# MAGIC-AI4Med/KEEP

Measured on AMD Instinct MI355X. Metric: 224x224 tiles encoded/sec (whole node), higher is better.
Workload: dtype fp16+mxfp4

## Files before the change

keep_amd/csrc/common.h:

```cpp
#pragma once
#include <hip/hip_runtime.h>
#include <stdint.h>

typedef _Float16 f16;
typedef _Float16 f16x2 __attribute__((ext_vector_type(2)));
typedef _Float16 f16x4 __attribute__((ext_vector_type(4)));
typedef _Float16 f16x8 __attribute__((ext_vector_type(8)));
typedef float f32x4 __attribute__((ext_vector_type(4)));
typedef float f32x16 __attribute__((ext_vector_type(16)));

#define KEEP_WAVE 64

__device__ __forceinline__ void split_f16(float x, f16& hi, f16& lo) {
    asm("" : "+v"(x));
    hi = (f16)x;
    lo = (f16)(x - (float)hi);
}

__device__ __forceinline__ unsigned char clip8_fixed(int v) {
    v >>= 22;
    return (unsigned char)(v < 0 ? 0 : (v > 255 ? 255 : v));
}
__device__ __forceinline__ float gelu_erf(float x) {
    return 0.5f * x * (1.0f + erff(x * 0.70710678118654752440f));
}

// ... 365 lines not shown
```

keep_amd/csrc/gemm_f16_v2.hip:

```cpp
#include "gemm_epilogue.h"
#include "quant4.h"

#ifndef KEEP_A_AUX
#define KEEP_A_AUX 0
#endif
#ifndef KEEP_W_AUX
#define KEEP_W_AUX 0
#endif
namespace keepk {

constexpr int V2_BM = 256, V2_BK = 32;

__device__ int g_swz_mask_dummy;
__device__ __forceinline__ int v2_swz(int row, int mask = 3) { return (row >> 2) & mask; }
__device__ __forceinline__ int v2_lds_off(int row, int chunk, int mask = 3) {
    return row * V2_BK + ((chunk ^ v2_swz(row, mask)) << 3);
}

template <int N> __device__ __forceinline__ void wait_vmcnt() { asm volatile("s_waitcnt vmcnt(%0)" ::"n"(N) : "memory"); }

typedef const __attribute__((address_space(1))) void* gptr_t;
typedef __attribute__((address_space(3))) void* lptr_t;

constexpr int v2_waves_per_simd(int BN, int WM, int WN) { return (V2_BM / WM / 32) * (BN / WN / 32) * 16 > 128 ? 1 : 2; }

typedef int v8i __attribute__((ext_vector_type(8)));
typedef unsigned u32x4 __attribute__((ext_vector_type(4)));
constexpr int V2_ST2 = 32768;
constexpr int V2_SC2 = 2048;
constexpr int V2_NST2 = 4;
constexpr int V2_SC2_BASE = V2_NST2 * V2_ST2;
constexpr int V2_G2 = 5;
constexpr int V2_PERS_LDS = 160 * 1024;
constexpr int V2_PERS_LDS_F16 = 96 * 1024 + 8 * 4608;

template <int BN, int WM, int WN, int NSTAGE, int EPI, int COMP = 0, bool PERS = false>
__global__ __launch_bounds__(WM * WN * 64, v2_waves_per_simd(BN, WM, WN))
void gemm_f16_v2_kernel(GemmParams p) {
    static_assert(!PERS || (BN == 256 && NSTAGE == 4 && COMP == 0 && (EPI == EPI_F16 || EPI == EPI_GELU_F16 || EPI == EPI_RESID_LS)),
                  "the persistent walk is written for the plain 256x256 / 4-stage kernel");
    constexpr int V2_THREADS = WM * WN * 64;
    constexpr int BM = V2_BM, BK = V2_BK;
    constexpr int TM = BM / WM / 32;
    constexpr int TN = BN / WN / 32;
    constexpr int SLOTS = BK / 8;
    constexpr int A_ROUNDS = BM * SLOTS / V2_THREADS;
    constexpr int B_ROUNDS = BN * SLOTS / V2_THREADS;
    constexpr int G = A_ROUNDS + B_ROUNDS;
    constexpr int BUF_ELEMS = (BM + BN) * BK;
    extern __shared__ __attribute__((aligned(16))) unsigned char smem_raw[];
    f16* lds = reinterpret_cast<f16*>(smem_raw);

    const int tid = threadIdx.x;
    const int lane = tid & 63;
    const int wave = __builtin_amdgcn_readfirstlane(tid >> 6);
    const int wm = wave / WN, wn = wave % WN;

    const int ntn = p.N / BN;
    const int mtn = (p.M + BM - 1) / BM;
// ... 16 lines not shown
            const int remw = ntn % BW, rr = t - full_tiles;
            tm_ = rr / remw; tn_ = (ntn / BW) * BW + (rr - tm_ * remw);
        }
    };
    int tm, tn;
    tile_of(bidx, tm, tn);
    int m0 = tm * BM;
    int n0 = tn * BN;

    const int swz_mask = (p.ablate & 4) ? 0 : 3;
    const int KT = p.K / BK;
    int a_off[A_ROUNDS], w_off[B_ROUNDS];
#pragma unroll
    for (int r = 0; r < A_ROUNDS; ++r) {
        const int L = r * V2_THREADS + tid;
        const int row = L / SLOTS, c = (L % SLOTS) ^ v2_swz(row, swz_mask);
        a_off[r] = row * BK + c * 8;
    }
#pragma unroll
    for (int r = 0; r < B_ROUNDS; ++r) {
        const int L = r * V2_THREADS + tid;
        const int row = L / SLOTS, c = (L % SLOTS) ^ v2_swz(row, swz_mask);
        w_off[r] = ((n0 & 255) + row) * BK + c * 8;
    }
    int64_t a_tile = (int64_t)(m0 >> 8) * KT * 8192;
    int64_t w_tile = (int64_t)(n0 >> 8) * KT * 8192;
    int tile_cur = bidx, m0_n = 0, n0_n = 0;
    int64_t a_tile_n = 0, w_tile_n = 0;
    bool has_next = false, first_tile = true;

    int kt0 = 0, ktiles = KT;
    if (EPI == EPI_PARTIAL) {
        const int per = (KT + p.ksplit - 1) / p.ksplit;
        kt0 = zsplit * per;
        ktiles = (kt0 + per < KT ? kt0 + per : KT) - kt0;
    }
    const int steps = ktiles * p.nseg;
// ... 41 lines not shown
        f16* sw = sa + BM * BK;
#pragma unroll
        for (int r = 0; r < A_ROUNDS; ++r) {
            unsigned o = (unsigned)a_off[r] * 2u;
            asm volatile("" : "+v"(o));
            __builtin_amdgcn_global_load_lds((gptr_t)(reinterpret_cast<const char*>(ab) + o), (lptr_t)(sa + (r * V2_THREADS + wave * 64) * 8), 16, 0, KEEP_A_AUX);
        }
#pragma unroll
        for (int r = 0; r < B_ROUNDS; ++r) {
            unsigned o = (unsigned)w_off[r] * 2u;
            asm volatile("" : "+v"(o));
            __builtin_amdgcn_global_load_lds((gptr_t)(reinterpret_cast<const char*>(wb) + o), (lptr_t)(sw + (r * V2_THREADS + wave * 64) * 8), 16, 0, KEEP_W_AUX);
        }
    };

    f32x16 acc[TN][TM];
    long long t_start = 0, t_first = 0, t_loop = 0;
#ifdef KEEP_DIAGNOSTICS
    if (p.ablate >> 8) {
        const long long wait = (long long)((blockIdx.x >> 3) & 3) * (p.ablate >> 8) * 1024, t0 = __builtin_readcyclecounter();
        while (__builtin_readcyclecounter() - t0 < wait) __builtin_amdgcn_s_sleep(8);
    }
#endif
    if (p.dbg) t_start = __builtin_readcyclecounter();
  for (;;) {
    if constexpr (PERS) {
        const int tnx = tile_cur + (int)gridDim.x;
        has_next = tnx < nwg;
        int tm2, tn2;
        tile_of(has_next ? tnx : tile_cur, tm2, tn2);
        m0_n = tm2 * BM; n0_n = tn2 * BN;
        a_tile_n = (int64_t)(m0_n >> 8) * KT * 8192;
        w_tile_n = (int64_t)(n0_n >> 8) * KT * 8192;
    }
    const int frow = lane & 31, fhi = lane >> 5;
    f16x8 fw0[TN] = {}, fa0[TM], fw1[TN] = {}, fa1[TM];
    auto read_frags = [&](int st, int ks, f16x8 (&fw)[TN], f16x8 (&fa)[TM]) {
        const f16* sa = lds + st * BUF_ELEMS;
        const f16* sw = sa + BM * BK;
#ifdef KEEP_DIAGNOSTICS
        if (!(p.ablate & 8))
#endif
#pragma unroll
        for (int i = 0; i < TN; ++i)
            fw[i] = *reinterpret_cast<const f16x8*>(sw + v2_lds_off(wn * (TN * 32) + i * 32 + frow, ks * 2 + fhi, swz_mask));
#pragma unroll
        for (int j = 0; j < TM; ++j)
            fa[j] = *reinterpret_cast<const f16x8*>(sa + v2_lds_off(wm * (TM * 32) + j * 32 + frow, ks * 2 + fhi, swz_mask));
    };
    constexpr int HM = (TN * TM == 8) ? 5 : TM;
    auto mfma_head = [&](const f16x8 (&fw)[TN], const f16x8 (&fa)[TM]) {
#pragma unroll
        for (int m = 0; m < HM; ++m)
            acc[m / TM][m % TM] = __builtin_amdgcn_mfma_f32_32x32x16_f16(fw[m / TM], fa[m % TM], acc[m / TM][m % TM], 0, 0, 0);
    };
    auto mfma_tail = [&](const f16x8 (&fw)[TN], const f16x8 (&fa)[TM]) {
#pragma unroll
        for (int m = HM; m < TN * TM; ++m)
            acc[m / TM][m % TM] = __builtin_amdgcn_mfma_f32_32x32x16_f16(fw[m / TM], fa[m % TM], acc[m / TM][m % TM], 0, 0, 0);
    };
    auto mfma_group = [&](const f16x8 (&fw)[TN], const f16x8 (&fa)[TM]) { mfma_head(fw, fa); mfma_tail(fw, fa); };
    const unsigned char* aq = nullptr; const unsigned char* wq = nullptr; const unsigned char* sq = nullptr;
    if constexpr (COMP != 0) {
        aq = p.a_q + (int64_t)(m0 >> 8) * KT * 8192;
        wq = p.w_q + (int64_t)(n0 >> 8) * KT * 8192;
        if constexpr (COMP == 1) sq = (wave < 4 ? p.a_sc + (int64_t)(m0 >> 8) * KT * 512 : p.w_sc + (int64_t)(n0 >> 8) * KT * 512 + 256) + (wave & 3) * 512;
        else sq = (wave < 4 ? p.a_sc + (int64_t)(m0 >> 8) * KT * 512 : p.w_sc + (int64_t)(n0 >> 8) * KT * 512) + (wave & 3) * 256;
    }
    const unsigned char* aq_run = aq; const unsigned char* wq_run = wq; const unsigned char* sq_run = sq;
    auto stage2 = [&](int, int buf) {
        unsigned char* sb = smem_raw + buf * V2_ST2;
        unsigned v4 = lane * 4;
        asm volatile("" : "+v"(v4));
#pragma unroll
        for (int r = 0; r < 2; ++r) {
            unsigned va = COMP == 1 ? (tid >> 8) * 8192 + (tid & 255) * 16 : tid * 16, vw = COMP == 1 ? va + 4096 : va;
// ... 12 lines not shown

    if (PERS && p.dbg && !first_tile) t_start = __builtin_readcyclecounter();
    if (!PERS || first_tile) {
#pragma unroll
        for (int t = 0; t < NSTAGE - 1; ++t)
            if (t < steps) stage(t, t);
        if (steps >= NSTAGE - 1) wait_vmcnt<G * (NSTAGE - 2)>(); else wait_vmcnt<0>();
        __builtin_amdgcn_s_barrier();
        if (p.dbg) t_first = __builtin_readcyclecounter();
        if (NSTAGE - 1 < steps) stage(NSTAGE - 1, NSTAGE - 1);
    } else {
        stage(3, 3);
        if (p.dbg) t_first = t_start;
    }
#pragma unroll
    for (int i = 0; i < TN; ++i)
#pragma unroll
        for (int j = 0; j < TM; ++j)
#pragma unroll
            for (int r = 0; r < 16; ++r) acc[i][j][r] = 0.f;
    read_frags(0, 0, fw0, fa0);

#define KEEP_STEADY_STEP(ISSUE)                                                                                                    \
    {                                                                                                                              \
                                                     \
        mfma_head(fw0, fa0);                                                                                                       \
        KEEP_PIN();                                                                                                                \
        read_frags(s % NSTAGE, 1, fw1, fa1);                                                                                       \
        KEEP_PIN();                                                                                                                \
        mfma_tail(fw0, fa0);                                                                                                       \
        KEEP_PIN();                                                                                                                \
        wait_vmcnt<G * (NSTAGE - 2)>();                                                                                            \
        asm volatile("s_waitcnt lgkmcnt(0)" ::: "memory");                                                                         \
        __builtin_amdgcn_s_barrier();                                                                                              \
        KEEP_PIN();                                                                                                                \
                                                      \
        mfma_head(fw1, fa1);                                                                                                       \
        KEEP_PIN();                                                                                                                \
        ISSUE;                                                                                                                     \
        read_frags((s + 1) % NSTAGE, 0, fw0, fa0);                                                                                 \
        KEEP_PIN();                                                                                                                \
        mfma_tail(fw1, fa1);                                                                                                       \
    }
    int s = 0;
    if constexpr (PRE || PERS) {
        for (; s < steps - NSTAGE; ++s) KEEP_STEADY_STEP(stage(s + NSTAGE, s % NSTAGE))
        if constexpr (PRE) KEEP_STEADY_STEP(stage2(0, 0))
        else KEEP_STEADY_STEP(stage_next(0, 0))
        ++s;
    } else {
        for (; s < steps - (NSTAGE - 1); ++s) KEEP_STEADY_STEP(if (s + NSTAGE < steps) stage(s + NSTAGE, s % NSTAGE))
    }
#undef KEEP_STEADY_STEP
#define KEEP_DRAIN_STEP(WAIT, AFTER)                                                                                               \
    {                                                                                                                              \
        mfma_head(fw0, fa0);                                                                                                       \
        KEEP_PIN();                                                                                                                \
        read_frags(s % NSTAGE, 1, fw1, fa1);                                                                                       \
        KEEP_PIN();                                                                                                                \
        mfma_tail(fw0, fa0);                                                                                                       \
        KEEP_PIN();                                                                                                                \
        wait_vmcnt<WAIT>();                                                                                                        \
        asm volatile("s_waitcnt lgkmcnt(0)" ::: "memory");                                                                         \
        __builtin_amdgcn_s_barrier();                                                                                              \
        KEEP_PIN();                                                                                                                \
        mfma_head(fw1, fa1);                                                                                                       \
        KEEP_PIN();                                                                                                                \
        AFTER;                                                                                                                     \
        read_frags((s + 1) % NSTAGE, 0, fw0, fa0);                                                                                 \
        KEEP_PIN();                                                                                                                \
        mfma_tail(fw1, fa1);                                                                                                       \
    }
    if constexpr (PRE) {
        KEEP_DRAIN_STEP(G + V2_G2, stage2(1, 1))
        ++s;
        KEEP_DRAIN_STEP(2 * V2_G2, stage2(2, 2))
        ++s;
    } else if constexpr (PERS) {
        KEEP_DRAIN_STEP(2 * G, stage_next(1, 1))
        ++s;
        KEEP_DRAIN_STEP(2 * G, stage_next(2, 2))
        ++s;
    } else {
        for (; s < steps - 1; ++s) KEEP_DRAIN_STEP(0, (void)0)
    }
#undef KEEP_DRAIN_STEP
    mfma_head(fw0, fa0);
    KEEP_PIN();
    read_frags(s % NSTAGE, 1, fw1, fa1);
    KEEP_PIN();
    mfma_tail(fw0, fa0);
    mfma_group(fw1, fa1);
#undef KEEP_PIN

    if constexpr (COMP != 0) {
        static_assert(BN == 256 && WM == 2 && WN == 4, "phase 2 is written for the 2 x 4 wave grid of the 256 x 256 tile");
        constexpr int G2 = V2_G2;
        if (p.dbg) t_first = __builtin_readcyclecounter();
        constexpr int FH = COMP == 1 ? 4096 : 8192;
        constexpr int SEC = COMP == 1 ? 8192 : 4096;
        constexpr int SFH = COMP == 1 ? 256 : 512, SSEC = COMP == 1 ? 512 : 256;
        const int NC = COMP == 1 ? p.K >> 7 : p.K >> 6;
        if constexpr (PRE) {
            wait_vmcnt<G2 * (V2_NST2 - 2)>();
            asm volatile("s_waitcnt lgkmcnt(0)" ::: "memory");
            __builtin_amdgcn_s_barrier();
        } else {
            asm volatile("s_waitcnt lgkmcnt(0)" ::: "memory");
            __builtin_amdgcn_s_barrier();
#pragma unroll
            for (int t = 0; t < V2_NST2 - 1; ++t)
                if (t < NC) stage2(t, t);
            if (NC >= V2_NST2 - 1) wait_vmcnt<G2 * (V2_NST2 - 2)>(); else wait_vmcnt<0>();
            __builtin_amdgcn_s_barrier();
        }
        const int a_row = (wm * 128 + frow) * 16, w_row = (wn * 64 + frow) * 16;
        const int asc_off = fhi * SFH + (wm * 32 + frow) * 4, wsc_off = 1024 + fhi * SFH + ((wn >> 1) * 32 + frow) * 4;
        const int wsh = (wn & 1) * 16;
#define KEEP_V8(V_) v8i{(int)(V_).x, (int)(V_).y, (int)(V_).z, (int)(V_).w, 0, 0, 0, 0}
#define KEEP_MX(I, J) \
            if constexpr (COMP == 1) { \
                acc[I][J] = __builtin_amdgcn_mfma_scale_f32_32x32x64_f8f6f4(KEEP_V8(wh[I]), KEEP_V8(ah[J]), acc[I][J], 4, 4, I, swh, J, sah); \
                acc[I][J] = __builtin_amdgcn_mfma_scale_f32_32x32x64_f8f6f4(KEEP_V8(wl[I]), KEEP_V8(al[J]), acc[I][J], 4, 4, I, swl, J, sal); \
            } else { \
                acc[I][J] = __builtin_amdgcn_mfma_scale_f32_32x32x64_f8f6f4(KEEP_V8(wl[I]), KEEP_V8(ah[J]), acc[I][J], 4, 4, I, swl, J, sah); \
                acc[I][J] = __builtin_amdgcn_mfma_scale_f32_32x32x64_f8f6f4(KEEP_V8(wh[I]), KEEP_V8(al[J]), acc[I][J], 4, 4, I, swh, J, sal); \
            }
#define KEEP_CHUNK(ISSUE, WAIT)                                                                                                    \
        {                                                                                                                          \
            const unsigned char* sb = smem_raw + (c & (V2_NST2 - 1)) * V2_ST2;                                                     \
            const unsigned char* ss = smem_raw + V2_SC2_BASE + (c & (V2_NST2 - 1)) * V2_SC2;                                       \
            const unsigned char* sa = sb + fhi * FH;         \
            const unsigned char* sw = sb + 16384 + fhi * FH;                                                                       \
                      \
              \
            u32x4 ah[4], al[4], wh[2], wl[2];                                                                                      \
            _Pragma("unroll") for (int jj = 0; jj < 4; ++jj) {                                                                     \
                ah[jj] = *reinterpret_cast<const u32x4*>(sa + a_row + jj * 512);                                                   \
                al[jj] = *reinterpret_cast<const u32x4*>(sa + SEC + a_row + jj * 512);                                             \
            }                                                                                                                      \
            _Pragma("unroll") for (int ii = 0; ii < 2; ++ii) {                                                                     \
                wh[ii] = *reinterpret_cast<const u32x4*>(sw + w_row + ii * 512);                                                   \
                wl[ii] = *reinterpret_cast<const u32x4*>(sw + SEC + w_row + ii * 512);                                             \
            }                                                                                                                      \
            const int sah = *reinterpret_cast<const int*>(ss + asc_off), sal = *reinterpret_cast<const int*>(ss + asc_off + SSEC); \
            const int swh = (int)(*reinterpret_cast<const unsigned*>(ss + wsc_off) >> wsh),                                        \
                      swl = (int)(*reinterpret_cast<const unsigned*>(ss + wsc_off + SSEC) >> wsh);                                 \
            ISSUE;                                                                     \
            KEEP_MX(0, 0) KEEP_MX(0, 1) KEEP_MX(0, 2) KEEP_MX(0, 3)                                                                \
            KEEP_MX(1, 0) KEEP_MX(1, 1) KEEP_MX(1, 2) KEEP_MX(1, 3)                                                                \
            wait_vmcnt<WAIT>();                                                                          \
            asm volatile("s_waitcnt lgkmcnt(0)" ::: "memory");                                                                     \
            __builtin_amdgcn_s_barrier();                                                                                          \
            __builtin_amdgcn_sched_barrier(0);               \
        }
        int c = 0;
        for (; c < NC - (V2_NST2 - 1); ++c) KEEP_CHUNK(stage2(c + V2_NST2 - 1, (c + V2_NST2 - 1) & (V2_NST2 - 1)), G2 * (V2_NST2 - 2))
#pragma clang loop unroll(disable)
        for (; c < NC; ++c) KEEP_CHUNK((void)0, 0)
#undef KEEP_CHUNK
#undef KEEP_MX
#undef KEEP_V8
    }

    if (p.dbg) t_loop = __builtin_readcyclecounter();

    if constexpr (EPI == EPI_TOP2) {
        const int C = p.top2_c;
        const int slot = (m0 >> 8) * 2 + wm;
        float* dst = p.top2_partial + (int64_t)slot * p.top2_kpad;
#pragma unroll
        for (int i = 0; i < TN; ++i)
#pragma unroll
            for (int rg = 0; rg < 4; ++rg) {
                float sa = 0.f, sb = 0.f;
#pragma unroll
                for (int j = 0; j < TM; ++j) {
                    const bool valid = m0 + wm * (TM * 32) + j * 32 + frow < p.M;
                    const float v0 = acc[i][j][rg * 4 + 0], v1 = acc[i][j][rg * 4 + 1], v2 = acc[i][j][rg * 4 + 2], v3 = acc[i][j][rg * 4 + 3];
                    const float a = fmaxf(v0, v1), b = fminf(v0, v1), c = fmaxf(v2, v3), d = fminf(v2, v3);
                    if (C == 4) {
                        const float t1 = fmaxf(a, c), t2 = fmaxf(fminf(a, c), fmaxf(b, d));
                        sa += valid ? (t1 - t2) - fabsf(t1 + t2 - 1.0f) : 0.f;
                    } else {
                        sa += valid ? (a - b) - fabsf(a + b - 1.0f) : 0.f;
                        sb += valid ? (c - d) - fabsf(c + d - 1.0f) : 0.f;
                    }
                }
#pragma unroll
                for (int o = 1; o < 32; o <<= 1) { sa += __shfl_xor(sa, o); sb += __shfl_xor(sb, o); }
                if (frow == 0) {
                    const int n = n0 + wn * (TN * 32) + i * 32 + 8 * rg + 4 * fhi;
                    if (C == 4) dst[n >> 2] = sa;
                    else { dst[n >> 1] = sa; dst[(n >> 1) + 1] = sb; }
                }
            }
        return;
    }
    __syncthreads();
    constexpr int WN_COLS = TN * 32;
    constexpr int PITCH = WN_COLS + 4;
    constexpr int PITCH16 = WN_COLS + 8;
    constexpr int SLAB_FLOATS = ((32 * PITCH > 32 * PITCH16 ? 32 * PITCH : 32 * PITCH16) + 63) / 64 * 64 + 96;
    static_assert(SLAB_FLOATS * 4 * WM * WN <= NSTAGE * (V2_BM + BN) * V2_BK * 2, "epilogue slabs must fit the LDS ring");
    constexpr int SLAB_BASE = PERS ? 3 * (V2_BM + BN) * V2_BK * 2 : 0;
    constexpr int SLAB_STRIDE = PERS ? ((EPI == EPI_F16 || EPI == EPI_GELU_F16) ? 1152 : 2048) : SLAB_FLOATS;
    static_assert(!PERS || (SLAB_BASE + SLAB_STRIDE * 4 * WM * WN <= V2_PERS_LDS && 32 * PITCH16 * 2 <= SLAB_STRIDE * 4), "persistent epilogue slabs must fit behind the three prefetched stages");
    float* slab = reinterpret_cast<float*>(smem_raw + SLAB_BASE) + wave * SLAB_STRIDE;
    auto slab_off = [&](int r, int col) { return PERS ? r * 64 + ((((col >> 2) + r) & 15) << 2) : r * PITCH + col; };
    const bool want_lo = !PERS && (p.out_lo || (p.out_q && COMP != 1));
    constexpr bool F16_OUT = (EPI == EPI_F16 || EPI == EPI_GELU_F16);
    constexpr int CPL = F16_OUT ? 8 : 4;
    constexpr int LPR = WN_COLS / CPL;
    constexpr int RPI = 64 / LPR;
    const int ocol = (lane % LPR) * CPL;
    const int orow_in = lane / LPR;
    const int ncol = n0 + wn * WN_COLS + ocol;
    f32x4 bias4[CPL / 4], ls4[CPL / 4];
#pragma unroll
    for (int c = 0; c < CPL / 4; ++c) {
        bias4[c] = (EPI == EPI_PARTIAL) ? f32x4{0.f, 0.f, 0.f, 0.f} : *reinterpret_cast<const f32x4*>(p.bias + ncol + c * 4);
        if (EPI == EPI_RESID_LS) ls4[c] = *reinterpret_cast<const f32x4*>(p.ls + ncol + c * 4);
    }
    f16* slab_hi = reinterpret_cast<f16*>(slab);
    f16* slab_lo = slab_hi + 32 * PITCH16;
    f32x4 bfrag[F16_OUT ? TN * 4 : 1];
    if (F16_OUT) {
#pragma unroll
        for (int i = 0; i < TN; ++i)
#pragma unroll
            for (int rg = 0; rg < 4; ++rg)
                bfrag[i * 4 + rg] = *reinterpret_cast<const f32x4*>(p.bias + n0 + wn * WN_COLS + i * 32 + 8 * rg + 4 * fhi);
    }
    f32x4 res2[2][32 / RPI];
    int64_t oo2[2][32 / RPI];
    auto load_res = [&](int jj, f32x4 (&res)[32 / RPI], int64_t (&oo)[32 / RPI]) {
        const int mb = m0 + wm * (TM * 32) + jj * 32;
#pragma unroll
        for (int it = 0; it < 32 / RPI; ++it) {
            const int m = mb + it * RPI + orow_in;
            const int mc = m < p.M ? m : p.M - 1;
            int prow; int64_t orow;
            gemm_epilogue_row<EPI>(p, mc, prow, orow);
            oo[it] = orow * p.N + ncol;
            if (EPI == EPI_PARTIAL) { oo[it] = ((int64_t)zsplit * p.M + mc) * p.N + ncol; res[it] = f32x4{0.f, 0.f, 0.f, 0.f}; }
            else if (EPI == EPI_PATCH) res[it] = *reinterpret_cast<const f32x4*>(p.pos + (int64_t)prow * p.N + ncol);
            else res[it] = __builtin_nontemporal_load(reinterpret_cast<const f32x4*>(p.resid + oo[it]));
        }
    };
    if (!F16_OUT) load_res(0, res2[0], oo2[0]);
    const int64_t out_sa = p.out_kt > 0 ? (int64_t)p.out_kt * 8192 : (int64_t)256 * p.N;
    const int out_sb = p.out_kt > 0 ? 32 : p.N;
    const int out_g = p.out_kt > 0 ? ((ncol >> 5) * 8192 + (ncol & 31)) : ncol;
#pragma unroll
    for (int j = 0; j < TM; ++j) {
        const int mbase = m0 + wm * (TM * 32) + j * 32;
        if (F16_OUT) {
#pragma unroll
            for (int i = 0; i < TN; ++i)
#pragma unroll
                for (int rg = 0; rg < 4; ++rg) {
                    f32x2 a = {acc[i][j][rg * 4 + 0] + bfrag[i * 4 + rg][0], acc[i][j][rg * 4 + 1] + bfrag[i * 4 + rg][1]};
                    f32x2 b = {acc[i][j][rg * 4 + 2] + bfrag[i * 4 + rg][2], acc[i][j][rg * 4 + 3] + bfrag[i * 4 + rg][3]};
                    if (EPI == EPI_GELU_F16) {
                        if (COMP != 0 || (!PERS && (p.out_lo || p.out_q))) { a = gelu_fast2(a); b = gelu_fast2(b); }
                        else { a = gelu_fast2_fp16(a); b = gelu_fast2_fp16(b); }
                    }
                    f16x4 h, l;
                    f16 hh, ll;
                    split_f16(a[0], hh, ll); h[0] = hh; l[0] = ll;
                    split_f16(a[1], hh, ll); h[1] = hh; l[1] = ll;
                    split_f16(b[0], hh, ll); h[2] = hh; l[2] = ll;
                    split_f16(b[1], hh, ll); h[3] = hh; l[3] = ll;
                    const int so = frow * PITCH16 + i * 32 + 8 * rg + 4 * fhi;
                    *reinterpret_cast<f16x4*>(slab_hi + so) = h;
                    if (want_lo) *reinterpret_cast<f16x4*>(slab_lo + so) = l;
                }
#pragma unroll
            for (int it = 0; it < 32 / RPI; ++it) {
                const int r = it * RPI + orow_in;
                const int m = mbase + r;
                const f16x8 h = *reinterpret_cast<const f16x8*>(slab_hi + r * PITCH16 + ocol);
                if (m < p.M) {
                    const int64_t o = (int64_t)(m >> 8) * out_sa + (m & 255) * out_sb + out_g;
                    __builtin_nontemporal_store(h, reinterpret_cast<f16x8*>(p.out_hi + o));
                    if (want_lo) {
                        const f16x8 l = *reinterpret_cast<const f16x8*>(slab_lo + r * PITCH16 + ocol);
                        if (p.out_lo) *reinterpret_cast<f16x8*>(p.out_lo + o) = l;
                        if (p.out_q) q4_store8(p.out_q, p.out_sc, p.out_kt, m, ncol >> 5, (ocol >> 3) & 3, h, l);
                    } else if (COMP == 1 && !PERS && p.out_q) {
                        q4_store8_hi(p.out_q, p.out_sc, p.out_kt, m, ncol >> 5, (ocol >> 3) & 3, h);
                    }
                }
            }
        } else {
#pragma unroll
            for (int i = 0; i < TN; ++i)
#pragma unroll
                for (int rg = 0; rg < 4; ++rg) {
                    f32x4 v;
#pragma unroll
                    for (int e = 0; e < 4; ++e) v[e] = acc[i][j][rg * 4 + e];
                    *reinterpret_cast<f32x4*>(slab + slab_off(frow, i * 32 + 8 * rg + 4 * fhi)) = v;
                }
            if (j + 1 < TM) load_res(j + 1, res2[(j + 1) & 1], oo2[(j + 1) & 1]);
#pragma unroll
            for (int it = 0; it < 32 / RPI; ++it) {
                const int r = it * RPI + orow_in;
                f32x4 x = *reinterpret_cast<const f32x4*>(slab + slab_off(r, ocol));
#pragma unroll
                for (int e = 0; e < 4; ++e) {
                    x[e] += bias4[0][e];
                    x[e] = (EPI == EPI_RESID_LS) ? res2[j & 1][it][e] + __fmul_rn(ls4[0][e], x[e]) : res2[j & 1][it][e] + x[e];
                }
                if (mbase + r < p.M) {
                    float* dst = (EPI == EPI_PARTIAL) ? p.splitk_ws : (EPI == EPI_RESID_F32) ? p.out_f32 : p.resid;
                    __builtin_nontemporal_store(x, reinterpret_cast<f32x4*>(dst + oo2[j & 1][it]));
                }
            }
// ... 95 lines not shown
```

keep_amd/csrc/op_api.hip:

```cpp
#include "handle.h"
#include "quant4.h"

namespace {

__global__ void clock_probe_kernel(long long* out, int spin_ticks) {
    if (threadIdx.x != 0) return;
    const long long r0 = (long long)__builtin_amdgcn_s_memrealtime(), c0 = (long long)__builtin_readcyclecounter();
    long long r1 = r0;
    while (r1 - r0 < spin_ticks) { __builtin_amdgcn_s_sleep(32); r1 = (long long)__builtin_amdgcn_s_memrealtime(); }
    const long long c1 = (long long)__builtin_readcyclecounter();
    out[0] = c1 - c0; out[1] = r1 - r0;
}

__global__ void f16_planes_to_f32_kernel(const f16* hi, const f16* lo, float* out, int64_t n) {
    for (int64_t i = (int64_t)blockIdx.x * blockDim.x + threadIdx.x; i < n; i += (int64_t)gridDim.x * blockDim.x)
        out[i] = (float)hi[i] + (lo ? (float)lo[i] : 0.f);
}
void planes_to_f32(const f16* hi, const f16* lo, float* out, int64_t n, hipStream_t s) {
    int blocks = (int)((n + 255) / 256); if (blocks > 4096) blocks = 4096; if (blocks < 1) blocks = 1;
    hipLaunchKernelGGL(f16_planes_to_f32_kernel, dim3(blocks), dim3(256), 0, s, hi, lo, out, n);
}

struct Planes { f16 *hi, *lo; unsigned char *q, *sc; };
Planes alloc_planes(Tmp& t, int64_t rows, int64_t K, bool fp4) {
// ... 34 lines not shown
    if (cls_out) { a.cls_hi = c_hi; a.cls_lo = c_lo; }
    if (kind == ATTN_OP_LONG ? launch_attention_long(a, s) : launch_attention(a, s)) return ATTN_REFUSED;
    launch_unblockify_f32(o_hi, split ? o_lo : nullptr, out, (int)M, (int)D, s);
    if (cls_out) launch_unblockify_f32(c_hi, c_lo, cls_out, (int)B, (int)D, s);
    HIPCHK(h, hipStreamSynchronize(s));
    return check_launch(h, what);
}

}

extern "C" {

int keep_op_linear(keep_handle* h, const float* a, const float* w, const float* bias, const float* ls, const float* resid,
                   int64_t M, int64_t N, int64_t K, int epi, int split, float* out, void* stream) {
    if (!h || !a || !w || !bias || !out) return h ? h->fail(KEEP_EINVAL, "null pointer") : KEEP_EINVAL;
    if (M < 1 || N % 128 || N < 128 || K < 64 || K % 32) return h->fail(KEEP_EUNSUPPORTED, "linear needs N%%128==0 and K%%32==0");
    if (epi != EPI_F16 && epi != EPI_GELU_F16 && epi != EPI_RESID_LS && epi != EPI_RESID_F32) return h->fail(KEEP_EINVAL, "epilogue %d", epi);
    if ((epi == EPI_RESID_LS && (!ls || !resid)) || (epi == EPI_RESID_F32 && !resid)) return h->fail(KEEP_EINVAL, "missing ls/resid");
    const bool comp = split == 2 || split == 3;
    if (comp && (N % 256 || K % 128 || K < (split == 3 ? 512 : 256) || epi == EPI_RESID_F32)) return h->fail(KEEP_EUNSUPPORTED, "compensated linear needs N%%256==0, K%%128==0, K>=256 (512 for the one-term form) and epilogue 0/1/2");
    KEEP_ON_DEVICE(h);
    hipStream_t s = (hipStream_t)stream;
    Tmp t;
    const Planes A = alloc_planes(t, M, K, comp), W = alloc_planes(t, N, K, comp), O = alloc_planes(t, M, N, false);
    float* ws = t.get<float>(SKINNY_WS_BYTES / 4);
    if (!t.ok) return h->fail(KEEP_ENOMEM, "temp alloc");
    if (comp) { launch_quant_blockify(a, A.hi, A.lo, A.q, A.sc, (int)M, (int)K, s); launch_quant_blockify(w, W.hi, W.lo, W.q, W.sc, (int)N, (int)K, s); }
    else { launch_split_blockify(a, A.hi, A.lo, (int)M, (int)K, s); launch_split_blockify(w, W.hi, W.lo, (int)N, (int)K, s); }
    GemmParams p = gemm_params(h, A.hi, A.lo, W.hi, W.lo, (int)M, (int)N, (int)K, split == 1, bias);
    p.ls = ls;
    if (comp) with_fp4(p, split == 3 ? 1 : 2, A, W);
    with_splitk(p, ws);
    int launch_rc = 0;
    if (epi == EPI_F16 || epi == EPI_GELU_F16) {
        p.out_hi = O.hi; p.out_lo = split ? O.lo : nullptr;
        p.out_kt = (epi == EPI_GELU_F16) ? (int)(N / 32) : 0;
        launch_rc = launch_gemm_f16(p, epi, s);
        if (p.out_kt) launch_unblockify_f32(O.hi, p.out_lo, out, (int)M, (int)N, s);
        else planes_to_f32(O.hi, p.out_lo, out, M * N, s);
    } else if (epi == EPI_RESID_LS) {
        HIPCHK(h, hipMemcpyAsync(out, resid, M * N * sizeof(float), hipMemcpyDeviceToDevice, s));
        p.resid = out;
        launch_rc = launch_gemm_f16(p, epi, s);
    } else {
        p.resid = const_cast<float*>(resid); p.out_f32 = out;
        launch_rc = launch_gemm_f16(p, epi, s);
    }
    HIPCHK(h, hipStreamSynchronize(s));
    if (launch_rc < 0) return h->fail(KEEP_EUNSUPPORTED, "op_linear: no kernel for this shape / mode");
    return check_launch(h, "op_linear");
}

int keep_op_linear_ln(keep_handle* h, const float* a, const float* w, const float* bias, const float* ls, const float* resid,
                      const float* ln_gamma, const float* ln_beta, float ln_eps, int64_t M, int64_t N, int64_t K, int epi, int split,
                      float* out, float* ln_out, float* ln_hi, int* did_ln, void* stream) {
    if (!h || !a || !w || !bias || !resid || !ln_gamma || !ln_beta || !out || !ln_out || !did_ln) return h ? h->fail(KEEP_EINVAL, "null pointer") : KEEP_EINVAL;
    if (M < 1 || (split != 0 && split != 1)) return h->fail(KEEP_EINVAL, "linear_ln needs M >= 1 and split 0 / 1");
// ... 158 lines not shown
    KEEP_ON_DEVICE(h);
    hipStream_t s = (hipStream_t)stream;
    const int64_t n = B * T * 3 * heads * 64;
    Tmp t;
    f16* q_hi = t.get<f16>(n); f16* q_lo = t.get<f16>(n);
    float* a_tmp = r_in ? t.get<float>((size_t)B * (q_rows ? 1 : T) * T) : nullptr;
    if (!t.ok) return h->fail(KEEP_ENOMEM, "temp alloc");
    launch_split_f16(qkv, q_hi, q_lo, n, s);
    if (launch_attention_rollout_step(q_hi, split ? q_lo : nullptr, (int)B, (int)T, heads, 0.125f, residual, r_in, r_out, q_rows, a_tmp, s))
        return h->fail(KEEP_EUNSUPPORTED, "attention_rollout_step: B %lld, T %lld, heads %d unsupported", (long long)B, (long long)T, heads);
    HIPCHK(h, hipStreamSynchronize(s));
    return check_launch(h, "op_attention_rollout_step");
}

__global__ __launch_bounds__(512, 2) void mfma_probe_kernel(const f16x8* __restrict__ src, float* __restrict__ sink, int iters) {
    f16x8 a[2], b[4];
    const int t = blockIdx.x * 512 + threadIdx.x;
#pragma unroll
    for (int i = 0; i < 2; ++i) a[i] = src[(size_t)t * 6 + i];
#pragma unroll
    for (int i = 0; i < 4; ++i) b[i] = src[(size_t)t * 6 + 2 + i];
    f32x16 acc[8];
#pragma unroll
    for (int i = 0; i < 8; ++i)
#pragma unroll
        for (int r = 0; r < 16; ++r) acc[i][r] = 0.f;
    for (int it = 0; it < iters; ++it) {
#pragma unroll
        for (int i = 0; i < 2; ++i)
#pragma unroll
            for (int j = 0; j < 4; ++j) acc[i * 4 + j] = __builtin_amdgcn_mfma_f32_32x32x16_f16(a[i], b[j], acc[i * 4 + j], 0, 0, 0);
    }
    float v = 0.f;
#pragma unroll
    for (int i = 0; i < 8; ++i)
#pragma unroll
        for (int r = 0; r < 16; ++r) v += acc[i][r];
    sink[t] = v;
}

int keep_op_layernorm(keep_handle* h, const float* x, const float* add, const float* gamma, const float* beta, int64_t rows,
                      int64_t D, float eps, float* out, void* stream) {
    if (!h || !x || !gamma || !beta || !out || rows < 1) return h ? h->fail(KEEP_EINVAL, "bad layernorm arguments") : KEEP_EINVAL;
    KEEP_ON_DEVICE(h);
    LnParams p = ln_params(h, x, D, (int)rows, (int)D, eps);
    p.add = add; p.gamma = gamma; p.beta = beta;
    p.out_f32 = out; p.out_f32_stride = D;
    if (launch_layernorm(p, (hipStream_t)stream)) return h->fail(KEEP_EUNSUPPORTED, "layernorm width %lld", (long long)D);
    return check_launch(h, "op_layernorm");
}

int keep_op_sgemm(keep_handle* h, const float* a, const float* b, const float* bias, int64_t M, int64_t N, int64_t K, float scale,
// ... 170 lines not shown
```

Measured before the change: 7187.

## Switch f16 GEMM main loop to 16x16x32 MFMA with matching LDS swizzle

Measured after the change: 7358 (median of 6 runs). +2.4%, better.

```diff
diff --git a/keep_amd/csrc/common.h b/keep_amd/csrc/common.h
--- a/keep_amd/csrc/common.h
+++ b/keep_amd/csrc/common.h
@@ -10,6 +10,11 @@
 typedef float f32x16 __attribute__((ext_vector_type(16)));
 
 #define KEEP_WAVE 64
+
+#ifndef KEEP_MFMA_SHAPE
+#define KEEP_MFMA_SHAPE 16
+#endif
+static_assert(KEEP_MFMA_SHAPE == 16 || KEEP_MFMA_SHAPE == 32, "KEEP_MFMA_SHAPE: 16 (16x16x32) or 32 (32x32x16)");
 
 __device__ __forceinline__ void split_f16(float x, f16& hi, f16& lo) {
     asm("" : "+v"(x));
diff --git a/keep_amd/csrc/gemm_f16_v2.hip b/keep_amd/csrc/gemm_f16_v2.hip
--- a/keep_amd/csrc/gemm_f16_v2.hip
+++ b/keep_amd/csrc/gemm_f16_v2.hip
@@ -7,14 +7,17 @@
 #ifndef KEEP_W_AUX
 #define KEEP_W_AUX 0
 #endif
+#ifndef KEEP_MFMA_HM16
+#define KEEP_MFMA_HM16 12
+#endif
 namespace keepk {
 
 constexpr int V2_BM = 256, V2_BK = 32;
 
 __device__ int g_swz_mask_dummy;
-__device__ __forceinline__ int v2_swz(int row, int mask = 3) { return (row >> 2) & mask; }
-__device__ __forceinline__ int v2_lds_off(int row, int chunk, int mask = 3) {
-    return row * V2_BK + ((chunk ^ v2_swz(row, mask)) << 3);
+template <int MS> __device__ __forceinline__ int v2_swz(int row, int mask = 3) { return (MS == 16 ? -(row >> 2) : (row >> 2)) & mask; }
+template <int MS> __device__ __forceinline__ int v2_lds_off(int row, int chunk, int mask = 3) {
+    return row * V2_BK + ((chunk ^ v2_swz<MS>(row, mask)) << 3);
 }
 
 template <int N> __device__ __forceinline__ void wait_vmcnt() { asm volatile("s_waitcnt vmcnt(%0)" ::"n"(N) : "memory"); }
@@ -23,6 +26,32 @@
 typedef __attribute__((address_space(3))) void* lptr_t;
 
 constexpr int v2_waves_per_simd(int BN, int WM, int WN) { return (V2_BM / WM / 32) * (BN / WN / 32) * 16 > 128 ? 1 : 2; }
+
+template <int MS> struct AccMap;
+template <> struct AccMap<32> {
+    typedef f32x16 acc_t;
+    static constexpr int ROW_LANES = 32;
+    static constexpr int QPG = 1;
+    __device__ static __forceinline__ int row(int q, int lane) { return lane & 31; }
+    __device__ static __forceinline__ int col(int q, int lane) { return (q >> 2) * 32 + (q & 3) * 8 + 4 * (lane >> 5); }
+    __device__ static __forceinline__ int colgroup(int q) { return q; }
+    __device__ static __forceinline__ int colgroup_col(int g, int lane) { return (g >> 2) * 32 + (g & 3) * 8 + 4 * (lane >> 5); }
+    template <class A> __device__ static __forceinline__ f32x4 quad(const A& acc, int pass, int q) {
+        const f32x16& v = acc[q >> 2][pass];
+        const int b = (q & 3) * 4;
+        return f32x4{v[b], v[b + 1], v[b + 2], v[b + 3]};
+    }
+};
+template <> struct AccMap<16> {
+    typedef f32x4 acc_t;
+    static constexpr int ROW_LANES = 16;
+    static constexpr int QPG = 2;
+    __device__ static __forceinline__ int row(int q, int lane) { return (q & 1) * 16 + (lane & 15); }
+    __device__ static __forceinline__ int col(int q, int lane) { return (q >> 1) * 16 + 4 * (lane >> 4); }
+    __device__ static __forceinline__ int colgroup(int q) { return q >> 1; }
+    __device__ static __forceinline__ int colgroup_col(int g, int lane) { return g * 16 + 4 * (lane >> 4); }
+    template <class A> __device__ static __forceinline__ f32x4 quad(const A& acc, int pass, int q) { return acc[q >> 1][2 * pass + (q & 1)]; }
+};
 
 typedef int v8i __attribute__((ext_vector_type(8)));
 typedef unsigned u32x4 __attribute__((ext_vector_type(4)));
@@ -41,8 +70,13 @@
                   "the persistent walk is written for the plain 256x256 / 4-stage kernel");
     constexpr int V2_THREADS = WM * WN * 64;
     constexpr int BM = V2_BM, BK = V2_BK;
+    constexpr int MS = COMP == 0 ? KEEP_MFMA_SHAPE : 32;
+    typedef AccMap<MS> Map;
     constexpr int TM = BM / WM / 32;
     constexpr int TN = BN / WN / 32;
+    constexpr int TMF = BM / WM / MS;
+    constexpr int TNF = BN / WN / MS;
+    constexpr int TAH = MS == 32 ? TMF : TMF / 2;
     constexpr int SLOTS = BK / 8;
     constexpr int A_ROUNDS = BM * SLOTS / V2_THREADS;
     constexpr int B_ROUNDS = BN * SLOTS / V2_THREADS;
@@ -89,13 +123,13 @@
 #pragma unroll
     for (int r = 0; r < A_ROUNDS; ++r) {
         const int L = r * V2_THREADS + tid;
-        const int row = L / SLOTS, c = (L % SLOTS) ^ v2_swz(row, swz_mask);
+        const int row = L / SLOTS, c = (L % SLOTS) ^ v2_swz<MS>(row, swz_mask);
         a_off[r] = row * BK + c * 8;
     }
 #pragma unroll
     for (int r = 0; r < B_ROUNDS; ++r) {
         const int L = r * V2_THREADS + tid;
-        const int row = L / SLOTS, c = (L % SLOTS) ^ v2_swz(row, swz_mask);
+        const int row = L / SLOTS, c = (L % SLOTS) ^ v2_swz<MS>(row, swz_mask);
         w_off[r] = ((n0 & 255) + row) * BK + c * 8;
     }
     int64_t a_tile = (int64_t)(m0 >> 8) * KT * 8192;
@@ -167,7 +201,7 @@
         }
     };
 
-    f32x16 acc[TN][TM];
+    typename Map::acc_t acc[TNF][TMF];
     long long t_start = 0, t_first = 0, t_loop = 0;
 #ifdef KEEP_DIAGNOSTICS
     if (p.ablate >> 8) {
@@ -187,32 +221,53 @@
         w_tile_n = (int64_t)(n0_n >> 8) * KT * 8192;
     }
     const int frow = lane & 31, fhi = lane >> 5;
-    f16x8 fw0[TN] = {}, fa0[TM], fw1[TN] = {}, fa1[TM];
-    auto read_frags = [&](int st, int ks, f16x8 (&fw)[TN], f16x8 (&fa)[TM]) {
+    const int foff16 = v2_lds_off<16>(lane & 15, lane >> 4, swz_mask);
+    f16x8 fw0[TNF] = {}, fa0[TAH], fw1[TNF] = {}, fa1[TAH];
+    f16x8 (&fwg1)[TNF] = MS == 32 ? fw1 : fw0;
+    f16x8 fwx = {};
+    auto read_frags = [&](int st, int g, f16x8 (&fw)[TNF], f16x8 (&fa)[TAH]) {
         const f16* sa = lds + st * BUF_ELEMS;
         const f16* sw = sa + BM * BK;
+        if constexpr (MS == 32) {
 #ifdef KEEP_DIAGNOSTICS
-        if (!(p.ablate & 8))
+            if (!(p.ablate & 8))
 #endif
 #pragma unroll
-        for (int i = 0; i < TN; ++i)
-            fw[i] = *reinterpret_cast<const f16x8*>(sw + v2_lds_off(wn * (TN * 32) + i * 32 + frow, ks * 2 + fhi, swz_mask));
-#pragma unroll
-        for (int j = 0; j < TM; ++j)
-            fa[j] = *reinterpret_cast<const f16x8*>(sa + v2_lds_off(wm * (TM * 32) + j * 32 + frow, ks * 2 + fhi, swz_mask));
+            for (int i = 0; i < TNF; ++i)
+                fw[i] = *reinterpret_cast<const f16x8*>(sw + v2_lds_off<MS>(wn * (TN * 32) + i * 32 + frow, g * 2 + fhi, swz_mask));
+#pragma unroll
+            for (int j = 0; j < TAH; ++j)
+                fa[j] = *reinterpret_cast<const f16x8*>(sa + v2_lds_off<MS>(wm * (TM * 32) + j * 32 + frow, g * 2 + fhi, swz_mask));
+        } else {
+            if (g == 0) {
+#ifdef KEEP_DIAGNOSTICS
+                if (!(p.ablate & 8))
+#endif
+#pragma unroll
+                for (int i = 0; i < TNF; ++i)
+                    (i < TNF - 1 ? fw[i] : fwx) = *reinterpret_cast<const f16x8*>(sw + (wn * (TN * 32) + i * 16) * BK + foff16);
+            } else {
+                fw0[TNF - 1] = fwx;
+            }
+#pragma unroll
+            for (int j = 0; j < TAH; ++j)
+                fa[j] = *reinterpret_cast<const f16x8*>(sa + (wm * (TM * 32) + (g * TAH + j) * 16) * BK + foff16);
+        }
     };
-    constexpr int HM = (TN * TM == 8) ? 5 : TM;
-    auto mfma_head = [&](const f16x8 (&fw)[TN], const f16x8 (&fa)[TM]) {
-#pragma unroll
-        for (int m = 0; m < HM; ++m)
-            acc[m / TM][m % TM] = __builtin_amdgcn_mfma_f32_32x32x16_f16(fw[m / TM], fa[m % TM], acc[m / TM][m % TM], 0, 0, 0);
+    constexpr int GM = TNF * TAH;
+    constexpr int HM = MS == 32 ? ((GM == 8) ? 5 : TAH) : ((GM == 16) ? KEEP_MFMA_HM16 : GM / 2);
+    constexpr int HM1 = MS == 32 ? HM : (TNF - 1) * TAH;
+    static_assert(HM <= HM1, "group 0's head runs before the last W fragment is moved into place");
+    auto mfma_range = [&](int g, int lo, int hi, const f16x8 (&fw)[TNF], const f16x8 (&fa)[TAH]) {
+#pragma unroll
+        for (int m = lo; m < hi; ++m) {
+            if constexpr (MS == 32) acc[m / TAH][m % TAH] = __builtin_amdgcn_mfma_f32_32x32x16_f16(fw[m / TAH], fa[m % TAH], acc[m / TAH][m % TAH], 0, 0, 0);
+            else acc[m / TAH][g * TAH + m % TAH] = __builtin_amdgcn_mfma_f32_16x16x32_f16(fw[m / TAH], fa[m % TAH], acc[m / TAH][g * TAH + m % TAH], 0, 0, 0);
+        }
     };
-    auto mfma_tail = [&](const f16x8 (&fw)[TN], const f16x8 (&fa)[TM]) {
-#pragma unroll
-        for (int m = HM; m < TN * TM; ++m)
-            acc[m / TM][m % TM] = __builtin_amdgcn_mfma_f32_32x32x16_f16(fw[m / TM], fa[m % TM], acc[m / TM][m % TM], 0, 0, 0);
-    };
-    auto mfma_group = [&](const f16x8 (&fw)[TN], const f16x8 (&fa)[TM]) { mfma_head(fw, fa); mfma_tail(fw, fa); };
+    auto mfma_head = [&](int g, const f16x8 (&fw)[TNF], const f16x8 (&fa)[TAH]) { mfma_range(g, 0, g ? HM1 : HM, fw, fa); };
+    auto mfma_tail = [&](int g, const f16x8 (&fw)[TNF], const f16x8 (&fa)[TAH]) { mfma_range(g, g ? HM1 : HM, GM, fw, fa); };
+    auto mfma_group = [&](int g, const f16x8 (&fw)[TNF], const f16x8 (&fa)[TAH]) { mfma_head(g, fw, fa); mfma_tail(g, fw, fa); };
     const unsigned char* aq = nullptr; const unsigned char* wq = nullptr; const unsigned char* sq = nullptr;
     if constexpr (COMP != 0) {
         aq = p.a_q + (int64_t)(m0 >> 8) * KT * 8192;
@@ -255,33 +310,33 @@
         if (p.dbg) t_first = t_start;
     }
 #pragma unroll
-    for (int i = 0; i < TN; ++i)
-#pragma unroll
-        for (int j = 0; j < TM; ++j)
-#pragma unroll
-            for (int r = 0; r < 16; ++r) acc[i][j][r] = 0.f;
+    for (int i = 0; i < TNF; ++i)
+#pragma unroll
+        for (int j = 0; j < TMF; ++j)
+#pragma unroll
+            for (int r = 0; r < MS * MS / 64; ++r) acc[i][j][r] = 0.f;
     read_frags(0, 0, fw0, fa0);
 
 #define KEEP_STEADY_STEP(ISSUE)                                                                                                    \
     {                                                                                                                              \
                                                      \
-        mfma_head(fw0, fa0);                                                                                                       \
+        mfma_head(0, fw0, fa0);                                                                                                    \
         KEEP_PIN();                                                                                                                \
         read_frags(s % NSTAGE, 1, fw1, fa1);                                                                                       \
         KEEP_PIN();                                                                                                                \
-        mfma_tail(fw0, fa0);                                                                                                       \
+        mfma_tail(0, fw0, fa0);                                                                                                    \
         KEEP_PIN();                                                                                                                \
         wait_vmcnt<G * (NSTAGE - 2)>();                                                                                            \
         asm volatile("s_waitcnt lgkmcnt(0)" ::: "memory");                                                                         \
         __builtin_amdgcn_s_barrier();                                                                                              \
         KEEP_PIN();                                                                                                                \
                                                       \
-        mfma_head(fw1, fa1);                                                                                                       \
+        mfma_head(1, fwg1, fa1);                                                                                                   \
         KEEP_PIN();                                                                                                                \
         ISSUE;                                                                                                                     \
         read_frags((s + 1) % NSTAGE, 0, fw0, fa0);                                                                                 \
         KEEP_PIN();                                                                                                                \
-        mfma_tail(fw1, fa1);                                                                                                       \
+        mfma_tail(1, fwg1, fa1);                                                                                                   \
     }
     int s = 0;
     if constexpr (PRE || PERS) {
@@ -295,22 +350,22 @@
 #undef KEEP_STEADY_STEP
 #define KEEP_DRAIN_STEP(WAIT, AFTER)                                                                                               \
     {                                                                                                                              \
-        mfma_head(fw0, fa0);                                                                                                       \
+        mfma_head(0, fw0, fa0);                                                                                                    \
         KEEP_PIN();                                                                                                                \
         read_frags(s % NSTAGE, 1, fw1, fa1);                                                                                       \
         KEEP_PIN();                                                                                                                \
-        mfma_tail(fw0, fa0);                                                                                                       \
+        mfma_tail(0, fw0, fa0);                                                                                                    \
         KEEP_PIN();                                                                                                                \
         wait_vmcnt<WAIT>();                                                                                                        \
         asm volatile("s_waitcnt lgkmcnt(0)" ::: "memory");                                                                         \
         __builtin_amdgcn_s_barrier();                                                                                              \
         KEEP_PIN();                                                                                                                \
-        mfma_head(fw1, fa1);                                                                                                       \
+        mfma_head(1, fwg1, fa1);                                                                                                   \
         KEEP_PIN();                                                                                                                \
         AFTER;                                                                                                                     \
         read_frags((s + 1) % NSTAGE, 0, fw0, fa0);                                                                                 \
         KEEP_PIN();                                                                                                                \
-        mfma_tail(fw1, fa1);                                                                                                       \
+        mfma_tail(1, fwg1, fa1);                                                                                                   \
     }
     if constexpr (PRE) {
         KEEP_DRAIN_STEP(G + V2_G2, stage2(1, 1))
@@ -326,12 +381,12 @@
         for (; s < steps - 1; ++s) KEEP_DRAIN_STEP(0, (void)0)
     }
 #undef KEEP_DRAIN_STEP
-    mfma_head(fw0, fa0);
+    mfma_head(0, fw0, fa0);
     KEEP_PIN();
     read_frags(s % NSTAGE, 1, fw1, fa1);
     KEEP_PIN();
-    mfma_tail(fw0, fa0);
-    mfma_group(fw1, fa1);
+    mfma_tail(0, fw0, fa0);
+    mfma_group(1, fwg1, fa1);
 #undef KEEP_PIN
 
     if constexpr (COMP != 0) {
@@ -361,20 +416,20 @@
 #define KEEP_V8(V_) v8i{(int)(V_).x, (int)(V_).y, (int)(V_).z, (int)(V_).w, 0, 0, 0, 0}
 #define KEEP_MX(I, J) \
             if constexpr (COMP == 1) { \
-                acc[I][J] = __builtin_amdgcn_mfma_scale_f32_32x32x64_f8f6f4(KEEP_V8(wh[I]), KEEP_V8(ah[J]), acc[I][J], 4, 4, I, swh, J, sah); \
-                acc[I][J] = __builtin_amdgcn_mfma_scale_f32_32x32x64_f8f6f4(KEEP_V8(wl[I]), KEEP_V8(al[J]), acc[I][J], 4, 4, I, swl, J, sal); \
+                acc[I][J] = __builtin_amdgcn_mfma_scale_f32_32x32x64_f8f6f4(KEEP_V8(wh[I]), KEEP_V8(ah[J]), acc[I][J], 4, 4, I, swh, J, sah);\
+                acc[I][J] = __builtin_amdgcn_mfma_scale_f32_32x32x64_f8f6f4(KEEP_V8(wl[I]), KEEP_V8(al[J]), acc[I][J], 4, 4, I, swl, J, sal);\
             } else { \
-                acc[I][J] = __builtin_amdgcn_mfma_scale_f32_32x32x64_f8f6f4(KEEP_V8(wl[I]), KEEP_V8(ah[J]), acc[I][J], 4, 4, I, swl, J, sah); \
-                acc[I][J] = __builtin_amdgcn_mfma_scale_f32_32x32x64_f8f6f4(KEEP_V8(wh[I]), KEEP_V8(al[J]), acc[I][J], 4, 4, I, swh, J, sal); \
+                acc[I][J] = __builtin_amdgcn_mfma_scale_f32_32x32x64_f8f6f4(KEEP_V8(wl[I]), KEEP_V8(ah[J]), acc[I][J], 4, 4, I, swl, J, sah);\
+                acc[I][J] = __builtin_amdgcn_mfma_scale_f32_32x32x64_f8f6f4(KEEP_V8(wh[I]), KEEP_V8(al[J]), acc[I][J], 4, 4, I, swh, J, sal);\
             }
 #define KEEP_CHUNK(ISSUE, WAIT)                                                                                                    \
         {                                                                                                                          \
             const unsigned char* sb = smem_raw + (c & (V2_NST2 - 1)) * V2_ST2;                                                     \
             const unsigned char* ss = smem_raw + V2_SC2_BASE + (c & (V2_NST2 - 1)) * V2_SC2;                                       \
-            const unsigned char* sa = sb + fhi * FH;         \
+            const unsigned char* sa = sb + fhi * FH;        \
             const unsigned char* sw = sb + 16384 + fhi * FH;                                                                       \
                       \
-              \
+             \
             u32x4 ah[4], al[4], wh[2], wl[2];                                                                                      \
             _Pragma("unroll") for (int jj = 0; jj < 4; ++jj) {                                                                     \
                 ah[jj] = *reinterpret_cast<const u32x4*>(sa + a_row + jj * 512);                                                   \
@@ -393,7 +448,7 @@
             wait_vmcnt<WAIT>();                                                                          \
             asm volatile("s_waitcnt lgkmcnt(0)" ::: "memory");                                                                     \
             __builtin_amdgcn_s_barrier();                                                                                          \
-            __builtin_amdgcn_sched_barrier(0);               \
+            __builtin_amdgcn_sched_barrier(0);              \
         }
         int c = 0;
         for (; c < NC - (V2_NST2 - 1); ++c) KEEP_CHUNK(stage2(c + V2_NST2 - 1, (c + V2_NST2 - 1) & (V2_NST2 - 1)), G2 * (V2_NST2 - 2))
@@ -411,14 +466,16 @@
         const int slot = (m0 >> 8) * 2 + wm;
         float* dst = p.top2_partial + (int64_t)slot * p.top2_kpad;
 #pragma unroll
-        for (int i = 0; i < TN; ++i)
-#pragma unroll
-            for (int rg = 0; rg < 4; ++rg) {
-                float sa = 0.f, sb = 0.f;
-#pragma unroll
-                for (int j = 0; j < TM; ++j) {
-                    const bool valid = m0 + wm * (TM * 32) + j * 32 + frow < p.M;
-                    const float v0 = acc[i][j][rg * 4 + 0], v1 = acc[i][j][rg * 4 + 1], v2 = acc[i][j][rg * 4 + 2], v3 = acc[i][j][rg * 4 + 3];
+        for (int cg = 0; cg < TN * 4 / Map::QPG; ++cg) {
+            float sa = 0.f, sb = 0.f;
+#pragma unroll
+            for (int j = 0; j < TM; ++j)
+#pragma unroll
+                for (int h = 0; h < Map::QPG; ++h) {
+                    const int q = cg * Map::QPG + h;
+                    const bool valid = m0 + wm * (TM * 32) + j * 32 + Map::row(q, lane) < p.M;
+                    const f32x4 v = Map::quad(acc, j, q);
+                    const float v0 = v[0], v1 = v[1], v2 = v[2], v3 = v[3];
                     const float a = fmaxf(v0, v1), b = fminf(v0, v1), c = fmaxf(v2, v3), d = fminf(v2, v3);
                     if (C == 4) {
                         const float t1 = fmaxf(a, c), t2 = fmaxf(fminf(a, c), fmaxf(b, d));
@@ -429,13 +486,13 @@
                     }
                 }
 #pragma unroll
-                for (int o = 1; o < 32; o <<= 1) { sa += __shfl_xor(sa, o); sb += __shfl_xor(sb, o); }
-                if (frow == 0) {
-                    const int n = n0 + wn * (TN * 32) + i * 32 + 8 * rg + 4 * fhi;
-                    if (C == 4) dst[n >> 2] = sa;
-                    else { dst[n >> 1] = sa; dst[(n >> 1) + 1] = sb; }
-                }
+            for (int o = 1; o < Map::ROW_LANES; o <<= 1) { sa += __shfl_xor(sa, o); sb += __shfl_xor(sb, o); }
+            if ((lane & (Map::ROW_LANES - 1)) == 0) {
+                const int n = n0 + wn * (TN * 32) + Map::colgroup_col(cg, lane);
+                if (C == 4) dst[n >> 2] = sa;
+                else { dst[n >> 1] = sa; dst[(n >> 1) + 1] = sb; }
             }
+        }
         return;
     }
     __syncthreads();
@@ -465,13 +522,13 @@
     }
     f16* slab_hi = reinterpret_cast<f16*>(slab);
     f16* slab_lo = slab_hi + 32 * PITCH16;
-    f32x4 bfrag[F16_OUT ? TN * 4 : 1];
+    constexpr int NQ = WN_COLS / 8;
+    constexpr int NCG = NQ / Map::QPG;
+    f32x4 bfrag[F16_OUT ? NCG : 1];
     if (F16_OUT) {
 #pragma unroll
-        for (int i = 0; i < TN; ++i)
-#pragma unroll
-            for (int rg = 0; rg < 4; ++rg)
-                bfrag[i * 4 + rg] = *reinterpret_cast<const f32x4*>(p.bias + n0 + wn * WN_COLS + i * 32 + 8 * rg + 4 * fhi);
+        for (int cg = 0; cg < NCG; ++cg)
+            bfrag[cg] = *reinterpret_cast<const f32x4*>(p.bias + n0 + wn * WN_COLS + Map::colgroup_col(cg, lane));
     }
     f32x4 res2[2][32 / RPI];
     int64_t oo2[2][32 / RPI];
@@ -498,11 +555,10 @@
         const int mbase = m0 + wm * (TM * 32) + j * 32;
         if (F16_OUT) {
 #pragma unroll
-            for (int i = 0; i < TN; ++i)
-#pragma unroll
-                for (int rg = 0; rg < 4; ++rg) {
-                    f32x2 a = {acc[i][j][rg * 4 + 0] + bfrag[i * 4 + rg][0], acc[i][j][rg * 4 + 1] + bfrag[i * 4 + rg][1]};
-                    f32x2 b = {acc[i][j][rg * 4 + 2] + bfrag[i * 4 + rg][2], acc[i][j][rg * 4 + 3] + bfrag[i * 4 + rg][3]};
+                for (int q = 0; q < NQ; ++q) {
+                    const f32x4 v = Map::quad(acc, j, q), bq = bfrag[Map::colgroup(q)];
+                    f32x2 a = {v[0] + bq[0], v[1] + bq[1]};
+                    f32x2 b = {v[2] + bq[2], v[3] + bq[3]};
                     if (EPI == EPI_GELU_F16) {
                         if (COMP != 0 || (!PERS && (p.out_lo || p.out_q))) { a = gelu_fast2(a); b = gelu_fast2(b); }
                         else { a = gelu_fast2_fp16(a); b = gelu_fast2_fp16(b); }
@@ -513,7 +569,7 @@
                     split_f16(a[1], hh, ll); h[1] = hh; l[1] = ll;
                     split_f16(b[0], hh, ll); h[2] = hh; l[2] = ll;
                     split_f16(b[1], hh, ll); h[3] = hh; l[3] = ll;
-                    const int so = frow * PITCH16 + i * 32 + 8 * rg + 4 * fhi;
+                    const int so = Map::row(q, lane) * PITCH16 + Map::col(q, lane);
                     *reinterpret_cast<f16x4*>(slab_hi + so) = h;
                     if (want_lo) *reinterpret_cast<f16x4*>(slab_lo + so) = l;
                 }
@@ -536,14 +592,8 @@
             }
         } else {
 #pragma unroll
-            for (int i = 0; i < TN; ++i)
-#pragma unroll
-                for (int rg = 0; rg < 4; ++rg) {
-                    f32x4 v;
-#pragma unroll
-                    for (int e = 0; e < 4; ++e) v[e] = acc[i][j][rg * 4 + e];
-                    *reinterpret_cast<f32x4*>(slab + slab_off(frow, i * 32 + 8 * rg + 4 * fhi)) = v;
-                }
+            for (int q = 0; q < NQ; ++q)
+                *reinterpret_cast<f32x4*>(slab + slab_off(Map::row(q, lane), Map::col(q, lane))) = Map::quad(acc, j, q);
             if (j + 1 < TM) load_res(j + 1, res2[(j + 1) & 1], oo2[(j + 1) & 1]);
 #pragma unroll
             for (int it = 0; it < 32 / RPI; ++it) {
diff --git a/keep_amd/csrc/op_api.hip b/keep_amd/csrc/op_api.hip
--- a/keep_amd/csrc/op_api.hip
+++ b/keep_amd/csrc/op_api.hip
@@ -72,7 +72,7 @@
 int keep_op_linear(keep_handle* h, const float* a, const float* w, const float* bias, const float* ls, const float* resid,
                    int64_t M, int64_t N, int64_t K, int epi, int split, float* out, void* stream) {
     if (!h || !a || !w || !bias || !out) return h ? h->fail(KEEP_EINVAL, "null pointer") : KEEP_EINVAL;
-    if (M < 1 || N % 128 || N < 128 || K < 64 || K % 32) return h->fail(KEEP_EUNSUPPORTED, "linear needs N%%128==0 and K%%32==0");
+    if (M < 1 || N % 128 || N < 128 || K < 32 || (K < 64 && h->tune.gemm_skinny_m > 0) || K % 32) return h->fail(KEEP_EUNSUPPORTED, "linear needs N%%128==0 and K%%32==0");
     if (epi != EPI_F16 && epi != EPI_GELU_F16 && epi != EPI_RESID_LS && epi != EPI_RESID_F32) return h->fail(KEEP_EINVAL, "epilogue %d", epi);
     if ((epi == EPI_RESID_LS && (!ls || !resid)) || (epi == EPI_RESID_F32 && !resid)) return h->fail(KEEP_EINVAL, "missing ls/resid");
     const bool comp = split == 2 || split == 3;
@@ -99,6 +99,7 @@
     } else if (epi == EPI_RESID_LS) {
         HIPCHK(h, hipMemcpyAsync(out, resid, M * N * sizeof(float), hipMemcpyDeviceToDevice, s));
         p.resid = out;
+        p.impl_hint = h->proj_impl;
         launch_rc = launch_gemm_f16(p, epi, s);
     } else {
         p.resid = const_cast<float*>(resid); p.out_f32 = out;
@@ -287,8 +288,10 @@
 }
 
 __global__ __launch_bounds__(512, 2) void mfma_probe_kernel(const f16x8* __restrict__ src, float* __restrict__ sink, int iters) {
+    const int t = blockIdx.x * 512 + threadIdx.x;
+    float v = 0.f;
+#if KEEP_MFMA_SHAPE == 32
     f16x8 a[2], b[4];
-    const int t = blockIdx.x * 512 + threadIdx.x;
 #pragma unroll
     for (int i = 0; i < 2; ++i) a[i] = src[(size_t)t * 6 + i];
 #pragma unroll
@@ -304,11 +307,35 @@
 #pragma unroll
             for (int j = 0; j < 4; ++j) acc[i * 4 + j] = __builtin_amdgcn_mfma_f32_32x32x16_f16(a[i], b[j], acc[i * 4 + j], 0, 0, 0);
     }
-    float v = 0.f;
 #pragma unroll
     for (int i = 0; i < 8; ++i)
 #pragma unroll
         for (int r = 0; r < 16; ++r) v += acc[i][r];
+#else
+    f16x8 a[8], b[4];
+    const int t2 = (t + 64) % ((int)gridDim.x * 512);
+#pragma unroll
+    for (int i = 0; i < 6; ++i) a[i] = src[(size_t)t * 6 + i];
+#pragma unroll
+    for (int i = 0; i < 2; ++i) a[6 + i] = src[(size_t)t2 * 6 + i];
+#pragma unroll
+    for (int i = 0; i < 4; ++i) b[i] = src[(size_t)t2 * 6 + 2 + i];
+    f32x4 acc[32];
+#pragma unroll
+    for (int i = 0; i < 32; ++i)
+#pragma unroll
+        for (int r = 0; r < 4; ++r) acc[i][r] = 0.f;
+    for (int it = 0; it < iters; it += 2) {
+#pragma unroll
+        for (int i = 0; i < 8; ++i)
+#pragma unroll
+            for (int j = 0; j < 4; ++j) acc[i * 4 + j] = __builtin_amdgcn_mfma_f32_16x16x32_f16(b[j], a[i], acc[i * 4 + j], 0, 0, 0);
+    }
+#pragma unroll
+    for (int i = 0; i < 32; ++i)
+#pragma unroll
+        for (int r = 0; r < 4; ++r) v += acc[i][r];
+#endif
     sink[t] = v;
 }
 
```
